# lastz/lastz

Measured on AMD Instinct MI355X. Metric: Gbp-of-target aligned/sec (whole job, --nogapped HSP path, both strands), higher is better.
Workload: dtype s32

## Files before the change

### lastz_amd/csrc/lz_lut.hpp

```cpp
#pragma once
#include "lz_common.hpp"

#define LZ_PAD2         128
#define LZ_LUT_ENTRIES  4096
#define LZ_LUT_TOTAL    (2 * LZ_LUT_ENTRIES)
#define LZ_LUT_WIN_G    15
#define LZ_LUT_WIN_B    60
#define LZ_LUT_MAXWIN   3
#define LZ_GRAY(c)      ((c) ^ ((c) >> 1))

struct alignas(8) LzLutEntry { u32 ab; u32 sc; };

struct LzLutParams {
    const u8* t2; const u8* q2;
    const u8* tsp; const u8* qsp;
    const u8* t2x; const u8* tspx;
    const u8* tcode; const u8* qcode;
    s32 xdrop;
};

struct LzLutScan { u32 s; s32 run, best; u32 room, used, alive, nwin; };

#if defined(__HIP_DEVICE_COMPILE__)
LZ_HD u32 lz_alignbit(u32 hi, u32 lo, u32 sh) { return __builtin_amdgcn_alignbit(hi, lo, sh); }
LZ_HD s32 lz_sdot4(u32 a, s32 acc) { return __builtin_amdgcn_sdot4((int)a, 0x01010101, acc, false); }
LZ_HD s32 lz_sdot4m(u32 a, u32 ones, s32 acc) { return __builtin_amdgcn_sdot4((int)a, (int)ones, acc, false); }
LZ_HD u32 lz_byte_pair(u32 hi_src, u32 lo_src, int k)
{ return __builtin_amdgcn_perm(hi_src, lo_src, 0x0C0C0000u | ((u32)(4 + k) << 8) | (u32)k); }
#define LZ_UNROLL_ALL _Pragma("unroll")
#else
LZ_HD u32 lz_alignbit(u32 hi, u32 lo, u32 sh) { sh &= 31u; return sh ? (lo >> sh) | (hi << (32u - sh)) : lo; }
LZ_HD s32 lz_sdot4(u32 a, s32 acc) { for (int k = 0; k < 4; k++) acc += (s32)(int8_t)(a >> (8 * k)); return acc; }
LZ_HD s32 lz_sdot4m(u32 a, u32 ones, s32 acc) { for (int k = 0; k < 4; k++) acc += (s32)(int8_t)(a >> (8 * k)) * (s32)((ones >> (8 * k)) & 0xFFu); return acc; }
LZ_HD u32 lz_byte_pair(u32 hi_src, u32 lo_src, int k) { return (((hi_src >> (8 * k)) & 0xFFu) << 8) | ((lo_src >> (8 * k)) & 0xFFu); }
#define LZ_UNROLL_ALL
#endif
LZ_HD u32 lz_ctz64(u64 x) { return (u32)__builtin_ctzll(x); }
LZ_HD u32 lz_clz64(u64 x) { return (u32)__builtin_clzll(x); }

template <bool SPECIAL> struct LzLutRaw { LzVec16 tv, qv, tm, qm; };
template <> struct LzLutRaw<false> { LzVec16 tv, qv; };
#define LZ_LUT_GBYTE(RIGHT_, g_) ((RIGHT_) ? (g_) : 14 - (g_))
template <bool RIGHT, bool SPECIAL>
LZ_HD void lz_lut_fetch(const LzLutParams& P, u32 s_, s32 diag, LzLutRaw<SPECIAL>& raw)
{
    const u32 st = RIGHT ? s_ + (u32)LZ_PAD2 : s_ - 1u + (u32)LZ_PAD2;
    const u32 sq = st - (u32)diag;
    const u32 back = RIGHT ? 0u : 15u;
    raw.tv = lz_load16(P.t2 + ((st >> 2) - back)); raw.qv = lz_load16(P.q2 + ((sq >> 2) - back));
    if constexpr (SPECIAL) {
        const u32 mback = RIGHT ? 0u : 14u;
        raw.tm = lz_load16(P.tsp + ((st >> 3) - mback)); raw.qm = lz_load16(P.qsp + ((sq >> 3) - mback));
    }
}
template <bool RIGHT>
LZ_HD u64 lz_lut_mask64(const LzVec16& v, s64 s)
{
    if (RIGHT) {
        const u32 k = (u32)((u64)(s + LZ_PAD2) & 7u);
        return ((u64)lz_alignbit(v.w[2], v.w[1], k) << 32) | lz_alignbit(v.w[1], v.w[0], k);
    }
    const u32 k = 17u + (u32)((u64)(s - 1 + LZ_PAD2) & 7u);
    return ((u64)lz_alignbit(v.w[3], v.w[2], k) << 32) | lz_alignbit(v.w[2], v.w[1], k);
}

template <bool RIGHT, bool SPECIAL, bool LIMCHK>
LZ_HD void lz_lut_window(const LzLutParams& P, const LzLutEntry* lut, s32 diag, LzLutScan& st, const LzLutRaw<SPECIAL>& raw, const s32* ctab = nullptr)
{
    const s32 X = P.xdrop;
    const LzLutEntry* const tab = lut + (RIGHT ? 0 : LZ_LUT_ENTRIES);
    const u32 spad = RIGHT ? st.s + (u32)LZ_PAD2 : st.s - 1u + (u32)LZ_PAD2, qpad = spad - (u32)diag;
    u32 tw[4], qw[4];
    {
        const u32 a = RIGHT ? 2u * (spad & 3u) : 2u * (spad & 3u) + 2u;
        const u32 b = RIGHT ? 2u * (qpad & 3u) : 2u * (qpad & 3u) + 2u;
        tw[0] = lz_alignbit(raw.tv.w[1], raw.tv.w[0], a); tw[1] = lz_alignbit(raw.tv.w[2], raw.tv.w[1], a); tw[2] = lz_alignbit(raw.tv.w[3], raw.tv.w[2], a); tw[3] = raw.tv.w[3] >> a;
        qw[0] = lz_alignbit(raw.qv.w[1], raw.qv.w[0], b); qw[1] = lz_alignbit(raw.qv.w[2], raw.qv.w[1], b); qw[2] = lz_alignbit(raw.qv.w[3], raw.qv.w[2], b); qw[3] = raw.qv.w[3] >> b;
    }
    u32 lim = st.room < (u32)LZ_LUT_WIN_B ? st.room : (u32)LZ_LUT_WIN_B;
    bool soft = false;
    if constexpr (SPECIAL) {
        const s64 s = (s64)st.s, sq = s - (s64)diag;
        const u64 sm = lz_lut_mask64<RIGHT>(raw.tm, s) | lz_lut_mask64<RIGHT>(raw.qm, sq);
        const u32 nsp = sm ? (RIGHT ? lz_ctz64(sm) : lz_clz64(sm)) : 64u;
        if (nsp < lim) { soft = true; lim = nsp; }
    }
    u32 xw[4], wc[4];
    LZ_UNROLL_ALL
    for (int k = 0; k < 4; k++) {
        xw[k] = tw[k] ^ qw[k];
        const u32 u = (tw[k] & 0x11111111u) | ((tw[k] >> 1) & 0x22222222u);
        wc[k] = (u | (u >> 2)) & 0x0F0F0F0Fu;
    }
    const u32 glim = lim >> 2;
    s32 run = st.run, m = run - st.best + X;
    u32 np = 0, fsc = 0;
#if !defined(LZ_LUT_NO_EARLY_EXIT) && defined(__HIP_DEVICE_COMPILE__)
    {
#define LZ_LUT_ENTRY_OF(g_) tab[lz_byte_pair(wc[LZ_LUT_GBYTE(RIGHT, g_) >> 2], xw[LZ_LUT_GBYTE(RIGHT, g_) >> 2], LZ_LUT_GBYTE(RIGHT, g_) & 3)]
        LzLutEntry ea = LZ_LUT_ENTRY_OF(0), eb = ea;
        LZ_UNROLL_ALL
        for (int g = 0; g < LZ_LUT_WIN_G; g += 2) {
            if (g + 1 < LZ_LUT_WIN_G) eb = LZ_LUT_ENTRY_OF(g + 1);
            if (m < (s32)(ea.ab & 0xFFFFu)) goto groups_done;
            if (LIMCHK && (u32)g >= glim) goto groups_done;
            { const s32 bq = (s32)ea.ab >> 16; m = lz_sdot4(ea.sc, m < bq ? m : bq); run = lz_sdot4(ea.sc, run); np = (u32)g + 1u; }
            if (g + 1 < LZ_LUT_WIN_G) {
                if (g + 2 < LZ_LUT_WIN_G) ea = LZ_LUT_ENTRY_OF(g + 2);
                if (m < (s32)(eb.ab & 0xFFFFu)) goto groups_done;
                if (LIMCHK && (u32)(g + 1) >= glim) goto groups_done;
                { const s32 bq = (s32)eb.ab >> 16; m = lz_sdot4(eb.sc, m < bq ? m : bq); run = lz_sdot4(eb.sc, run); np = (u32)g + 2u; }
            }
        }
        groups_done:
        fsc = (np & 1u) ? eb.sc : ea.sc;
#undef LZ_LUT_ENTRY_OF
    }
#else
    {
        bool dead = false;
        LZ_UNROLL_ALL
        for (int g = 0; g < LZ_LUT_WIN_G; g++) {
            const int by = LZ_LUT_GBYTE(RIGHT, g);
            const LzLutEntry e = tab[lz_byte_pair(wc[by >> 2], xw[by >> 2], by & 3)];
            if (!dead) fsc = e.sc;
            dead = dead | (m < (s32)(e.ab & 0xFFFFu));
            if (LIMCHK) dead = dead | ((u32)g >= glim);
            const s32 bq = (s32)e.ab >> 16;
            const s32 t = lz_sdot4(e.sc, m < bq ? m : bq);
            const s32 r2 = lz_sdot4(e.sc, run);
            m = dead ? m : t; run = dead ? run : r2; np += dead ? 0u : 1u;
        }
    }
#endif
    u32 r = 0;
    if (np < (u32)LZ_LUT_WIN_G) { r = lim - 4u * np; if (r > 4u) r = 4u; }
    s32 best = run - m + X;
    const u32 sc = fsc;
    bool stop = false; u32 j = 0;
    if (LIMCHK) {
        LZ_UNROLL_ALL
        for (u32 b = 0; b < 4; b++) {
            const bool on = !stop && b < r;
            const s32 nr = run + (s32)(int8_t)(sc >> (8u * b));
            run = on ? nr : run;
// ... 48 lines not shown
    diag = (s32)(u32)(key >> 32);
    const u32 pos1 = pos2 + (u32)diag;
    const s32 stopl = diag > 0 ? diag : 0;
    const s32 stopr = ((s32)tlen <= (s32)qlen + diag) ? (s32)tlen : (s32)qlen + diag;
    L.s = R.s = pos1; L.run = L.best = R.run = R.best = 0; L.used = R.used = 0; L.nwin = R.nwin = 0;
    L.room = (u32)((s32)pos1 - stopl); R.room = (u32)(stopr - (s32)pos1);
    L.alive = ((s32)pos1 > stopl) ? 1u : 0u; R.alive = ((s32)pos1 < stopr) ? 1u : 0u;
}

LZ_HD u32 lz_lut_summary(const LzLutScan& L, const LzLutScan& R, s32 min_score)
{
    u32 summ = (L.used & 0xFFu) | ((R.used & 0xFFu) << 8);
    if (L.alive || R.alive || L.best + R.best >= min_score) summ |= LZ_SUMM_SLOW;
    return summ;
}

template <bool SPECIAL>
LZ_HD u32 lz_lut_probe_hit(const LzLutParams& P, const LzLutEntry* lut, u32 tlen, u32 qlen, s32 min_score, u64 key, const s32* ctab = nullptr)
{
    s32 diag; LzLutScan L, R;
    lz_lut_init(key, tlen, qlen, diag, L, R);
    while (L.alive == 1 && L.nwin < (u32)LZ_LUT_MAXWIN) lz_lut_step<false, SPECIAL>(P, lut, diag, L, ctab);
    while (R.alive == 1 && R.nwin < (u32)LZ_LUT_MAXWIN) lz_lut_step<true, SPECIAL>(P, lut, diag, R, ctab);
    return lz_lut_summary(L, R, min_score);
}

LZ_HD u64 lz_hit_record(u64 key, u32 summ)
{
    const u32 pos2 = (u32)key, diag = (u32)(key >> 32);
    const bool slow = (summ & LZ_SUMM_SLOW) != 0;
    const u64 payload = slow ? (u64)(diag >> 16) : (u64)(summ & 0xFFFFu);
    return (u64)pos2 | ((u64)(diag & 0xFFu) << 31) | (payload << 39) | (slow ? (1ull << 63) : 0ull);
}
#define LZ_REC_TAG(r)     ((u32)((r) >> 55) & 0xFFu)
#define LZ_REC_UNTAG(r)   ((r) & ~(0xFFull << 55))
LZ_HD u64 lz_hit_record_tagged(u64 key, u32 summ) { return lz_hit_record(key, summ) | ((u64)((u32)(key >> 40) & 0xFFu) << 55); }

#define LZ_WCTX_BYTES 32
struct alignas(16) LzWctx { u32 w[LZ_WCTX_BYTES / 4]; };
LZ_HD u32 lz_wctx_first_byte(u32 pos1) { return ((pos1 - 1u + (u32)LZ_PAD2) >> 2) - 15u; }
LZ_HD u32 lz_wctx_right_offset(u32 pos1) { return ((pos1 + (u32)LZ_PAD2) >> 2) - lz_wctx_first_byte(pos1); }
LZ_HD LzWctx lz_wctx_make(const u8* two, u32 pos1) { LzWctx e; __builtin_memcpy(&e, two + lz_wctx_first_byte(pos1), LZ_WCTX_BYTES); return e; }
LZ_HD void lz_wctx_windows(const LzWctx& e, u32 pos1, LzVec16& tl, LzVec16& tr)
{
    const bool at16 = lz_wctx_right_offset(pos1) == 16u;
    LZ_UNROLL_ALL
    for (int k = 0; k < 4; k++) {
        tl.w[k] = e.w[k];
        const u32 at15 = lz_alignbit(e.w[4 + k], e.w[3 + k], 24u);
        tr.w[k] = at16 ? e.w[4 + k] : at15;
    }
}

#define LZ_REC_POS2(r)    ((u32)((r) & 0x7FFFFFFFu))
#define LZ_REC_LOW8(r)    ((u32)((r) >> 31) & 0xFFu)
#define LZ_REC_PAYLOAD(r) ((u32)((r) >> 39) & 0xFFFFu)
#define LZ_REC_SLOW(r)    ((u32)((r) >> 63))
LZ_HD u64 lz_rec_with_index(u64 r, u32 idx)
{ return (r & ~((0xFFull << 31) | (0x1Full << 55))) | ((u64)(idx & 0xFFu) << 31) | ((u64)((idx >> 8) & 0x1Fu) << 55); }
#define LZ_REC_INDEX(r)   (((u32)((r) >> 31) & 0xFFu) | (((u32)((r) >> 55) & 0x1Fu) << 8))

template <class Emit>
LZ_HD void lz_settle_record(const LzExtendParams& P, const s32* score_tab, u64 rec, u32 h ,
                            u32& dend, u64& n_ext, u64& n_bp, Emit&& emit)
{
    const u32 p2 = LZ_REC_POS2(rec);
    if (dend > p2 - P.seed_len) return;
    n_ext++;
    const u32 pay = LZ_REC_PAYLOAD(rec);
    if (!LZ_REC_SLOW(rec)) {
        const u32 room = p2 - dend, dlo = pay & 0xFFu, dext = pay >> 8;
        const u32 extent = p2 + dext;
        n_bp += (dlo < room ? dlo : room) + dext;
        if (extent > dend) dend = extent;
        return;
    }
    const s32 diag = (s32)((pay << 16) | h);
    dend = lz_reextend(P, score_tab, p2, diag, dend, n_bp, emit);
}
```

### lastz_amd/csrc/lzgpu_api.hip

```cpp
#include <hip/hip_runtime.h>
#include <stdarg.h>
#include <stdio.h>
#include <stdlib.h>
#include <string.h>
#include <math.h>
#include <algorithm>
#include <mutex>
#include <thread>
#include <atomic>
#include "lz_ctx.hpp"
#include "lz_host.hpp"
#include "lz_lut.hpp"


static LzCtx g_ctx;
static void lz_release_statics();
void lz_phase_clocks_print();
LzCtx& lz_ctx() { return g_ctx; }

static thread_local std::string t_last_error, t_last_error_out;
static std::mutex g_err_m;
int lz_fail(int code, const char* fmt, ...)
{
    char buf[512];
// ... 399 lines not shown
{
    LzCtx& c = g_ctx;
    if (!c.target.have_raw || !c.wstart.p) return lz_fail(LZGPU_ERR_STATE, "no table buffers");
    dev_ptr[0] = c.target.raw_base(); bytes[0] = c.geom.tlen;
    dev_ptr[1] = c.wstart.p;          bytes[1] = ((uint64_t)(1u << c.seed.weight) + 1) * 4;
    dev_ptr[2] = c.wpos.p;            bytes[2] = (uint64_t)c.num_words * 4;
    return 0;
}

extern "C" int lzgpu_table_commit(void)
{
    LzCtx& c = g_ctx;
    if (!c.target.have_raw || !c.wstart.p) return lz_fail(LZGPU_ERR_STATE, "no table buffers");
    { int rc = lz_bind_thread(); if (rc) return rc; }
    if (c.target.host.size() != c.geom.tlen) {
        c.target.host.resize(c.geom.tlen);
        if (c.geom.tlen) LZ_HIP(hipMemcpy(c.target.host.data(), c.target.raw_base(), c.geom.tlen, hipMemcpyDeviceToHost));
        c.target.code_key = 0; c.target.dp_key = 0;
    }
    c.table_gen++;
    c.have_table = true;
    return 0;
}

extern "C" int lzgpu_device_copy(void* dst, const void* src, uint64_t bytes)
{
    int rc = require_init(); if (rc) return rc;
    if (!bytes) return 0;
    LZ_HIP(hipMemcpyAsync(dst, src, bytes, hipMemcpyDeviceToDevice, g_ctx.stream));
    LZ_HIP(hipStreamSynchronize(g_ctx.stream));
    return 0;
}


#include <chrono>
struct HostProf {
    bool on; double t[16]; const char* names[16] = { nullptr }; int n = 0;
    std::chrono::steady_clock::time_point last;
    HostProf() { on = getenv("LZGPU_HOSTPROF") != nullptr; for (auto& x : t) x = 0; }
    void start() { if (on) last = std::chrono::steady_clock::now(); }
    void lap(int k, const char* name) {
        if (!on) return;
        auto now = std::chrono::steady_clock::now();
        t[k] += std::chrono::duration<double, std::milli>(now - last).count(); names[k] = name; if (k >= n) n = k + 1; last = now;
    }
    ~HostProf() { if (on) for (int k = 0; k < n; k++) if (names[k]) fprintf(stderr, "[lzgpu hostprof] %-28s %10.2f ms total\n", names[k], t[k]); }
};
static HostProf g_hp;


static int lz_wctx_prepare(LzCtx& c, bool& fused)
{
    if (c.wctx.p && c.wctx_gen == c.table_gen && c.wctx_code_key == c.target.code_key && c.target.code_key) return 0;
    const size_t need = (size_t)c.num_words * LZ_WCTX_BYTES;
    if (c.num_words == 0) { fused = false; return 0; }
    if (need > c.wctx.cap || !c.wctx.p) {
        size_t fr = 0, tot = 0;
        if (hipMemGetInfo(&fr, &tot) != hipSuccess || need > (fr + c.wctx.cap) / 2 || c.wctx.ensure(need) != 0) {
            (void)hipGetLastError(); c.last_error.clear();
            c.wctx_gen = 0; c.wctx_code_key = 0;
            fused = false;
            return 0;
        }
    }
    c.wctx_gen = 0; c.wctx_code_key = 0;
    int rc = lzk_wctx_build(c);
    if (rc) return rc;
    c.wctx_gen = c.table_gen; c.wctx_code_key = c.target.code_key;
    return 0;
}

static int seed_search(const lz_search_args* a, lz_hsp** out, uint64_t* n_out)
{
    int rc = require_init(); if (rc) return rc;
    LzCtx& c = g_ctx;
    if (!a || !out || !n_out || !a->sub) return lz_fail(LZGPU_ERR_ARG, "null argument");
    *out = nullptr; *n_out = 0;
    if (!c.have_table) return lz_fail(LZGPU_ERR_STATE, "lzgpu_table_prepare has not been called");

    g_hp.start();
    SeqSlot* qs;
    if (a->query) {
        if (a->qlen >= 0x7FFFFFFFu) return LZGPU_NH_SIZE;
        qs = lz_query_slot(c, -1, true);
        if ((rc = slot_upload(c, *qs, a->query, a->qlen, false))) return rc;
    } else {
        qs = a->query_slot < 0 ? nullptr : lz_query_slot(c, a->query_slot, false);
        if (!qs) return lz_fail(LZGPU_ERR_ARG, "query slot %d is empty", a->query_slot);
    }
    const u8* qhost = a->query ? a->query : qs->host.data();
    const u32 qlen = qs->len;
    u32 lo = a->start, hi = a->end ? a->end : qlen;
    if (hi <= lo) return lz_fail(LZGPU_ERR_ARG, "in seed_hit_search(), interval is void (%u-%u)", lo, hi);
    if (hi > qlen) return lz_fail(LZGPU_ERR_ARG, "in seed_hit_search(), interval end is bad (%u>%u)", hi, qlen);

    g_hp.lap(7, "query slot");
    static std::vector<s32> last_sub; static u8 rowc[256], colc[256]; static s32 tab[LZ_NCLASS * LZ_NCLASS];
    u8 cls[256];
    if (last_sub.size() != 65536 || memcmp(last_sub.data(), a->sub, 65536 * sizeof(s32)) != 0 || !c.score_tab.p) {
        last_sub.clear();
        if ((rc = lzh_score_classes(a->sub, rowc, colc, tab))) return rc;
        if ((rc = c.score_tab.ensure(sizeof(tab)))) return rc;
        LZ_HIP(hipMemcpyAsync(c.score_tab.p, tab, sizeof(tab), hipMemcpyHostToDevice, c.stream));
        LZ_HIP(hipStreamSynchronize(c.stream));
        last_sub.assign(a->sub, a->sub + 65536);
    }
    g_hp.lap(8, "score classes + table upload");
// ... 363 lines not shown
```

### lastz_amd/csrc/seed_kernels.hip

```cpp
#include <hip/hip_runtime.h>
#include <cstring>
#include <cstdio>
#include <rocprim/device/device_radix_sort.hpp>
#include <rocprim/device/device_scan.hpp>
#include <rocprim/iterator/transform_iterator.hpp>
#include "lz_ctx.hpp"
#include "lz_lut.hpp"
#include "lz_tile_runs.hpp"
#include "lz_coop.hpp"

#define LZ_TPB 256

#if defined(LZ_NO_NT)
#define LZ_NT_LD(p_) (*(p_))
#define LZ_NT_ST(v_, p_) (*(p_) = (v_))
#else
#define LZ_NT_LD(p_) __builtin_nontemporal_load(p_)
#define LZ_NT_ST(v_, p_) __builtin_nontemporal_store((v_), (p_))
#endif
__global__ void __launch_bounds__(LZ_TPB)
k_encode(const u8* __restrict__ raw, u8* __restrict__ code, u32 len, const u8* __restrict__ cls)
{
    __shared__ u8 tab[256];
    tab[threadIdx.x] = cls[threadIdx.x];
// ... 673 lines not shown
    bin_base[threadIdx.x] = bb;
    for (u32 b = 0; b < nblocks; b++) part[(size_t)b * LZ_NBIN + threadIdx.x] += bb;
}

int lzk_hist_scan(LzCtx& c, u64 n, u32* hist, u32* part, u32* bin_base, hipStream_t st)
{
    const u32 ntiles = (u32)((n + LZ_PP_TILE - 1) / LZ_PP_TILE), nblocks = (ntiles + 255u) / 256u;
    c.timer.begin("k_hist_scan", st);
    if (nblocks) hipLaunchKernelGGL(k_hist_scan1, dim3(nblocks), dim3(LZ_NBIN), 0, st, hist, ntiles, part);
    hipLaunchKernelGGL(k_hist_scan2, dim3(1), dim3(LZ_NBIN), 0, st, part, nblocks, bin_base);
    c.timer.end(st);
    LZ_HIP(hipGetLastError());
    return 0;
}

__device__ __forceinline__ void lz_match8(u32 key, bool valid, u32 lane, u32& rank, u32& count, bool& last)
{
    u64 peers = __ballot(valid);
#pragma unroll
    for (int b = 0; b < 8; b++) {
        const bool bit = ((key >> b) & 1u) != 0;
        const u64 m = __ballot(bit && valid);
        peers &= bit ? m : ~m;
    }
    const u64 below = (1ull << lane) - 1ull;
    rank = (u32)__popcll(peers & below);
    count = (u32)__popcll(peers);
    last = (peers >> lane) == 1ull;
}
__device__ __forceinline__ u32 lz_exscan256(u32 v, u32* wtot )
{
    const u32 tid = threadIdx.x, lane = tid & 63u, w = tid >> 6;
    u32 inc = v;
#pragma unroll
    for (int d = 1; d < 64; d <<= 1) { const u32 t = __shfl_up(inc, d); if ((int)lane >= d) inc += t; }
    if (tid < 256 && lane == 63) wtot[w] = inc;
    __syncthreads();
    u32 pre = 0;
    if (tid < 256) for (u32 k = 0; k < w; k++) pre += wtot[k];
    return pre + inc - v;
}

struct LzScanTask { u32 idx; s32 diag; LzLutScan L, R; };
static_assert(sizeof(LzScanTask) == 64, "LzScanTask: one 64-byte line per task");
#define LZ_SC_TPB 512
template <int MODE> struct LzScanShared {
    union {
        LzLutEntry lut[LZ_LUT_TOTAL];
        struct { s32 tab[LZ_NCLASS * LZ_NCLASS]; s32 tab8[64]; } bc;
    };
    s32 ctab[MODE == 1 ? LZ_NCLASS * LZ_NCLASS : 1];
};

template <bool SP>
__device__ __forceinline__ void lz_scan_round(const LzExtendParams& P, const LzLutParams& Q, const LzLutEntry* lut, const s32* ctab, u64 key, bool valid,
                                              const LzLutRaw<SP>& rawl, const LzLutRaw<SP>& rawr, u32 idx, u32 lane,
                                              u32& summ_out, LzScanTask* __restrict__ my_tasks, u32& my_n, u32 region_cap)
{
    constexpr bool HLIM = SP;
    s32 diag; LzLutScan L, R;
    lz_lut_init(key, P.tlen, P.qlen, diag, L, R);
    if (!valid) { L.alive = 0; R.alive = 0; }
    const bool ql = L.alive && !HLIM && L.room < (u32)LZ_LUT_WIN_B, qr = R.alive && !HLIM && R.room < (u32)LZ_LUT_WIN_B;
    lz_lut_window_pair<SP, HLIM>(Q, lut, diag, L, R, rawl, rawr, L.alive && !ql, R.alive && !qr, ctab);
    const bool more = valid && (L.alive == 1 || R.alive == 1);
    const u64 mm = __ballot(more);
    bool queued = false;
    if (mm) {
        const u32 slot = my_n + (u32)__popcll(mm & ((1ull << lane) - 1ull));
        if (more && slot < region_cap) {
            LzScanTask t; t.idx = idx; t.diag = diag; t.L = L; t.R = R;
            my_tasks[slot] = t; queued = true;
        }
        my_n += (u32)__popcll(mm);
    }
    summ_out = queued ? 0u : lz_lut_summary(L, R, P.min_score);
}
template <bool SP>
__device__ __forceinline__ void lz_scan_fetch(const LzLutParams& Q, u64 key, LzLutRaw<SP>& rawl, LzLutRaw<SP>& rawr)
{
    const u32 pos2 = (u32)key, pos1 = pos2 + (u32)(key >> 32);
    const s32 diag = (s32)(u32)(key >> 32);
    const u32 stl = pos1 - 1u + (u32)LZ_PAD2, str = pos1 + (u32)LZ_PAD2;
    const u32 bl = (stl >> 2) - 15u, br = str >> 2;
    const u32 ol = bl + (bl & ~31u);
    rawl.tv = lz_load16(Q.t2x + ol); rawr.tv = lz_load16(Q.t2x + (ol + (br - bl)));
    const u32 sql = stl - (u32)diag, sqr = str - (u32)diag;
    rawl.qv = lz_load16(Q.q2 + ((sql >> 2) - 15u)); rawr.qv = lz_load16(Q.q2 + (sqr >> 2));
    if constexpr (SP) {
        const u32 ml = (stl >> 3) - 14u, mr = str >> 3;
        const u32 oml = ml + (ml & ~31u);
        rawl.tm = lz_load16(Q.tspx + oml); rawr.tm = lz_load16(Q.tspx + (oml + (mr - ml)));
        rawl.qm = lz_load16(Q.qsp + ((sql >> 3) - 14u)); rawr.qm = lz_load16(Q.qsp + (sqr >> 3));
    }
}

template <int MODE, int TPB, int WPE>
__global__ void __launch_bounds__(TPB, WPE)
k_scan_hits(LzExtendParams P, LzLutParams Q, const u64* __restrict__ keys, u64 n,
            const s32* __restrict__ score_tab_g, const LzLutEntry* __restrict__ lut_g,
            u32* __restrict__ summ, u8* __restrict__ bins, LzScanTask* __restrict__ tasks, u32* __restrict__ n_tasks, u32 region_cap)
{
    __shared__ LzScanShared<MODE> sh;
    const u32 tid = threadIdx.x, lane = tid & 63u, w = tid >> 6;
    if (MODE == 1) { for (u32 k = tid; k < LZ_NCLASS * LZ_NCLASS; k += TPB) sh.ctab[k] = score_tab_g[k]; }
    if (MODE < 2) { for (u32 k = tid; k < LZ_LUT_TOTAL; k += TPB) sh.lut[k] = lut_g[k]; }
    else {
        for (u32 k = tid; k < LZ_NCLASS * LZ_NCLASS; k += TPB) sh.bc.tab[k] = score_tab_g[k];
        if (tid < 64) sh.bc.tab8[tid] = score_tab_g[(tid >> 3) * LZ_NCLASS + (tid & 7)];
    }
    __syncthreads();
    const LzLutEntry* lut = sh.lut;
    const s32* const ctab = sh.ctab;
    constexpr bool SP = MODE == 1;
    constexpr u32 SPAN = 64u * LZ_SC_ROUNDS;
    static_assert(LZ_SC_ROUNDS == 4, "the round pipeline below is written out for four rounds per span");
// ... 190 lines not shown
    if ((rc = c.summ[set].ensure((size_t)max_n * 4))) return rc;
    if (mode < 2 && (rc = c.scan_tasks[set].ensure((size_t)n_regions * region_cap * sizeof(LzScanTask)))) return rc;
    return c.scan_ntasks[set].ensure((size_t)n_regions * 4);
}

int lzk_scan_hits(LzCtx& c, int set, int mode, const LzExtendParams& P, const LzLutParams& Q, const u64* keys, u64 n,
                  const s32* score_tab, const LzLutEntry* lut, u8* bins, hipStream_t st)
{
    if (n == 0) return 0;
    int cus = 256; (void)hipDeviceGetAttribute(&cus, hipDeviceAttributeMultiprocessorCount, c.device);
    int rc;
    u32 grid, n_regions, task_cap;
    lz_scan_geometry(c, mode, n, grid, n_regions, task_cap);
    if ((rc = c.summ[set].ensure((size_t)n * 4))) return rc;
    if (mode < 2 && (rc = c.scan_tasks[set].ensure((size_t)n_regions * task_cap * sizeof(LzScanTask)))) return rc;
    if ((rc = c.scan_ntasks[set].ensure((size_t)n_regions * 4))) return rc;
    u32* summ = c.summ[set].as<u32>(); LzScanTask* tasks = c.scan_tasks[set].as<LzScanTask>(); u32* ntk = c.scan_ntasks[set].as<u32>();
    c.timer.begin("k_scan_hits", st);
    const int tpb = lz_scan_tpb(mode);
#define LZ_SCAN_LAUNCH(M_, T_, W_) hipLaunchKernelGGL((k_scan_hits<M_, T_, W_>), dim3(grid), dim3(T_), 0, st, P, Q, keys, n, score_tab, lut, summ, bins, tasks, ntk, task_cap)
    if (mode == 0) {
        if (tpb == 640)       LZ_SCAN_LAUNCH(0, 640, 5);
        else if (tpb == 768)  LZ_SCAN_LAUNCH(0, 768, 6);
        else if (tpb == 1024) LZ_SCAN_LAUNCH(0, 1024, 8);
        else                  LZ_SCAN_LAUNCH(0, 512, 4);
    }
    else if (mode == 1) LZ_SCAN_LAUNCH(1, LZ_SC_TPB, 4);
    else                LZ_SCAN_LAUNCH(2, LZ_SC_TPB, 4);
#undef LZ_SCAN_LAUNCH
    c.timer.end(st);
    LZ_HIP(hipGetLastError());
    if (mode < 2) {
        c.timer.begin("k_scan_tasks", st);
        if (mode == 0) hipLaunchKernelGGL(k_scan_tasks<0>, dim3(std::min<u32>(n_regions, 4u * (u32)cus)), dim3(LZ_ST_TPB), 0, st, P, Q, lut, score_tab, tasks, ntk, n_regions, task_cap, summ);
        else           hipLaunchKernelGGL(k_scan_tasks<1>, dim3(std::min<u32>(n_regions, 4u * (u32)cus)), dim3(LZ_ST_TPB), 0, st, P, Q, lut, score_tab, tasks, ntk, n_regions, task_cap, summ);
        c.timer.end(st);
        LZ_HIP(hipGetLastError());
    }
    return 0;
}

int lzk_partition(LzCtx& c, int set, u64* keys, u64 n, u32* hist, u32* run_addr, hipStream_t st)
{
    if (n == 0) return 0;
    const u32 ntiles = (u32)((n + LZ_PP_TILE - 1) / LZ_PP_TILE);
    c.timer.begin("k_partition", st);
    hipLaunchKernelGGL(k_partition, dim3(ntiles), dim3(LZ_PP_TPB), 0, st, keys, c.summ[set].as<u32>(), n, hist, run_addr, keys);
    c.timer.end(st);
    LZ_HIP(hipGetLastError());
    return 0;
}

__global__ void __launch_bounds__(LZ_TPB)
k_build_wctx(const u32* __restrict__ wpos, u64 num_words, const u8* __restrict__ two, LzVec16* __restrict__ wctx)
{
    const u64 j = (u64)blockIdx.x * LZ_TPB + threadIdx.x;
    if (j >= 2 * num_words) return;
    const u32 pos1 = wpos[j >> 1];
    wctx[j] = lz_load16(two + lz_wctx_first_byte(pos1) + 16u * (u32)(j & 1u));
}

template <int CAP> struct LzFuse2Wave {
    alignas(16) u32 own32[CAP / 2];
    u32 lsrc[64 * LZ_FILL_GROUP];
    uint2 ent[64];
};
struct LzFuseTrip { u32 p1, pos2, dst; bool ok; LzWctx cx; LzVec16 ql, qr; };

template <bool SELF, int TPB, int CAP>
__global__ void __launch_bounds__(TPB)
k_scan_hits2(u32 lo, u32 i0, u32 i1, LzSeedDev sd,
             const u32* __restrict__ wstart, const u32* __restrict__ wpos, const LzWctx* __restrict__ wctx,
             const u32* __restrict__ sk, const u32* __restrict__ sv, u32 n, const u64* __restrict__ off, u64 base,
             LzExtendParams P, LzLutParams Q, const LzLutEntry* __restrict__ lut_g,
             u64* __restrict__ recs, LzScanTask* __restrict__ tasks, u32* __restrict__ n_tasks, u32 region_cap, LzSelfDev self)
{
    static_assert(CAP % 512 == 0, "whole 16-byte groups of own[] per lane");
    constexpr int WORDS = CAP / 2 / 64;
    __shared__ LzLutEntry lut[LZ_LUT_TOTAL];
    __shared__ LzFuse2Wave<CAP> shw[TPB / 64];
    for (u32 k = threadIdx.x; k < LZ_LUT_TOTAL; k += TPB) lut[k] = lut_g[k];
    __syncthreads();
    LzFuse2Wave<CAP>& sh = shw[threadIdx.x >> 6];
    unsigned short* const own = reinterpret_cast<unsigned short*>(sh.own32);
    const u32 lane = threadIdx.x & 63u;
    const u32 region = blockIdx.x * (TPB / 64) + (threadIdx.x >> 6), nwaves = gridDim.x * (TPB / 64);
    LzScanTask* const my_tasks = tasks + (size_t)region * region_cap;
    u32 my_n = 0;
    const u32 ngroups = (n + 63u) / 64u;
    for (u32 grp = region; grp < ngroups; grp += nwaves) {
        const u32 j = grp * 64u + lane;
        u32 w_l = 0, i_l = 0; bool in = false;
        if (j < n) { w_l = sk[j] & ((2u << sd.weight) - 1u); i_l = sv[j]; in = !(w_l >> sd.weight) && i_l >= i0 && i_l < i1; }
        if (!__ballot(in)) continue;
        const u32 dbase = in ? (u32)(off[i_l] - base) : 0u;
        const u32 pos2 = lo + i_l + 1u;
        u32 slo = 0, shi = 0;
        if (SELF) lz_self_bounds(self, pos2, slo, shi);
        u32 carry = 0;
        for (int r = 0; r < sd.nprobes; r += LZ_FILL_GROUP) {
            u32 la[LZ_FILL_GROUP], len[LZ_FILL_GROUP]; u32 total = 0;
#pragma unroll
            for (int p = 0; p < LZ_FILL_GROUP; p++) {
                const bool on = in && r + p < sd.nprobes;
                const u32 w = on ? (w_l ^ sd.probe_xor[(r + p) & (LZ_MAX_PROBES - 1)]) : 0u;
                la[p] = wstart[w]; len[p] = wstart[w + 1];
            }
#pragma unroll
            for (int p = 0; p < LZ_FILL_GROUP; p++) {
                const bool on = in && r + p < sd.nprobes;
                len[p] = on ? len[p] - la[p] : 0u;
                if (!SELF) total += len[p];
            }
            if (SELF) {
                lz_clip_runs<LZ_FILL_GROUP>(wpos, la, len, slo, shi);
#pragma unroll
                for (int p = 0; p < LZ_FILL_GROUP; p++) total += len[p];
            }
            u32 inc = total;
            LZ_WAVE_SCAN_U32(inc, total, lz_uadd)
            const u32 E = inc - total;
            const u32 T = (u32)__builtin_amdgcn_readlane((int)inc, 63);
            {
                u32 S = E;
#pragma unroll
                for (int p = 0; p < LZ_FILL_GROUP; p++) { sh.lsrc[lane * LZ_FILL_GROUP + p] = la[p] - S; S += len[p]; }
            }
            sh.ent[lane] = make_uint2(dbase + carry - E, pos2);
            for (u32 cs = 0; cs < T; cs += CAP) {
                const u32 tc = (T - cs < (u32)CAP) ? T - cs : (u32)CAP;
                uint4* const mine = reinterpret_cast<uint4*>(sh.own32 + lane * WORDS);
#pragma unroll
                for (int k = 0; k < WORDS / 4; k++) mine[k] = make_uint4(0u, 0u, 0u, 0u);
                __atomic_signal_fence(__ATOMIC_SEQ_CST);
                {
                    u32 S = E;
#pragma unroll
                    for (int p = 0; p < LZ_FILL_GROUP; p++) {
                        const u32 l = len[p];
                        if (l && S < cs + tc && S + l > cs) own[(S > cs ? S : cs) - cs] = (unsigned short)(1u + lane * LZ_FILL_GROUP + (u32)p);
                        S += l;
                    }
                }
                __atomic_signal_fence(__ATOMIC_SEQ_CST);
                u32 wv[WORDS];
#pragma unroll
                for (int k = 0; k < WORDS / 4; k++) { const uint4 v = mine[k]; wv[4 * k] = v.x; wv[4 * k + 1] = v.y; wv[4 * k + 2] = v.z; wv[4 * k + 3] = v.w; }
                u32 segmax = 0;
#pragma unroll
                for (int k = 0; k < WORDS; k++) { const u32 m2 = lz_umax(wv[k] & 0xFFFFu, wv[k] >> 16); segmax = lz_umax(segmax, m2); }
                u32 sinc = segmax;
                LZ_WAVE_SCAN_U32(sinc, segmax, lz_umax)
                u32 run = lz_dpp_u32<0x138, 0xf, 0xf>(0u, sinc);
#pragma unroll
                for (int k = 0; k < WORDS; k++) {
                    const u32 a0 = lz_umax(wv[k] & 0xFFFFu, run), a1 = lz_umax(wv[k] >> 16, a0);
                    wv[k] = a0 | (a1 << 16); run = a1;
                }
#pragma unroll
                for (int k = 0; k < WORDS / 4; k++) mine[k] = make_uint4(wv[4 * k], wv[4 * k + 1], wv[4 * k + 2], wv[4 * k + 3]);
                __atomic_signal_fence(__ATOMIC_SEQ_CST);
                auto load_trip = [&](u32 tb, LzFuseTrip& t) {
                    const u32 t0 = tb + lane;
                    t.ok = t0 < tc;
                    const u32 tt = t.ok ? t0 : tc - 1u;
                    const u32 list = (u32)own[tt] - 1u;
                    const u32 ls = sh.lsrc[list];
                    const uint2 en = sh.ent[list / LZ_FILL_GROUP];
                    const u32 tabs = cs + tt, e = ls + tabs;
                    t.p1 = wpos[e]; t.cx = wctx[e];
                    t.pos2 = en.y; t.dst = en.x + tabs;
                    const u32 sql = en.y - 1u + (u32)LZ_PAD2;
                    t.ql = lz_load16(Q.q2 + ((sql >> 2) - 15u)); t.qr = lz_load16(Q.q2 + ((sql + 1u) >> 2));
                };
                auto scan_trip = [&](const LzFuseTrip& t) {
                    const u64 key = lz_hit_key(t.p1, t.pos2);
                    LzLutRaw<false> rl, rr;
                    lz_wctx_windows(t.cx, t.p1, rl.tv, rr.tv);
                    rl.qv = t.ql; rr.qv = t.qr;
                    u32 summ;
                    lz_scan_round<false>(P, Q, lut, nullptr, key, t.ok, rl, rr, t.dst, lane, summ, my_tasks, my_n, region_cap);
                    if (t.ok) LZ_NT_ST(lz_hit_record_tagged(key, summ), recs + t.dst);
                };
                LzFuseTrip ta, tb2;
                load_trip(0u, ta);
#pragma unroll 1
                for (u32 tb = 0;;) {
                    if (tb + 64u < tc) load_trip(tb + 64u, tb2);
                    scan_trip(ta);
                    tb += 64u; if (tb >= tc) break;
                    if (tb + 64u < tc) load_trip(tb + 64u, ta);
                    scan_trip(tb2);
                    tb += 64u; if (tb >= tc) break;
                }
                __atomic_signal_fence(__ATOMIC_SEQ_CST);
            }
            carry += total;
        }
    }
    if (lane == 0) n_tasks[region] = my_n < region_cap ? my_n : region_cap;
}

__global__ void __launch_bounds__(LZ_ST_TPB)
k_scan_tasks2(LzExtendParams P, LzLutParams Q, const LzLutEntry* __restrict__ lut_g, const LzScanTask* __restrict__ tasks,
              const u32* __restrict__ n_tasks, u32 n_regions, u32 region_cap, u64* __restrict__ recs)
{
    __shared__ LzLutEntry lut[LZ_LUT_TOTAL];
    for (u32 k = threadIdx.x; k < LZ_LUT_TOTAL; k += LZ_ST_TPB) lut[k] = lut_g[k];
    __syncthreads();
    for (u32 region = blockIdx.x; region < n_regions; region += gridDim.x) {
        const u32 nt = n_tasks[region];
        for (u32 k = threadIdx.x; k < nt; k += (u32)LZ_ST_TPB) {
            const LzScanTask t = tasks[(size_t)region * region_cap + k];
            LzLutScan L = t.L, R = t.R;
            const u32 pos1 = L.alive == 1 ? L.s + (u32)LZ_LUT_WIN_B * L.nwin : R.s - (u32)LZ_LUT_WIN_B * R.nwin;
            while (L.alive == 1 && L.nwin < (u32)LZ_LUT_MAXWIN) lz_lut_step<false, false>(Q, lut, t.diag, L, nullptr);
            while (R.alive == 1 && R.nwin < (u32)LZ_LUT_MAXWIN) lz_lut_step<true, false>(Q, lut, t.diag, R, nullptr);
            recs[t.idx] = lz_hit_record_tagged(lz_hit_key(pos1, pos1 - (u32)t.diag), lz_lut_summary(L, R, P.min_score));
        }
    }
}

__global__ void __launch_bounds__(LZ_PP_TPB)
k_partition2(u64* recs, u64 n, u32* __restrict__ hist, u32* __restrict__ run_addr)
{
    __shared__ LzPartShared sh;
    const u32 tid = threadIdx.x, lane = tid & 63u, w = tid >> 6;
    const u32 tile = blockIdx.x;
    const u64 base = (u64)tile * LZ_PP_TILE;
    const u32 tile_n = (n - base < (u64)LZ_PP_TILE) ? (u32)(n - base) : (u32)LZ_PP_TILE;
    for (u32 k = tid; k < LZ_PP_WAVES * LZ_NBIN; k += LZ_PP_TPB) { (&sh.wcnt[0][0])[k] = 0; (&sh.bm[0][0])[k] = 0ull; }
    const u32 l0 = w * (64u * LZ_PP_ROUNDS) + lane;
    u64 rr[LZ_PP_ROUNDS];
#pragma unroll
    for (u32 r = 0; r < LZ_PP_ROUNDS; r++) rr[r] = (l0 + 64u * r < tile_n) ? recs[base + l0 + 64u * r] : 0ull;
    __syncthreads();
#define LZ_PART_BIN(r_) LZ_REC_TAG(rr[r_])
    LZ_PART_RANKS(LZ_PART_BIN)
#undef LZ_PART_BIN
#pragma unroll
    for (u32 r = 0; r < LZ_PP_ROUNDS; r++) {
        const u32 bin = LZ_REC_TAG(rr[r]);
        if (l0 + 64u * r < tile_n) sh.stage[sh.tstart[bin] + sh.wcnt[w][bin] + slot[r]] = rr[r];
    }
    __syncthreads();
    lz_part_store(sh.stage, tile_n, recs + base);
}

int lzk_wctx_build(LzCtx& c)
{
    const u64 nw = c.num_words;
    if (nw == 0) return 0;
    c.timer.begin("k_build_wctx", c.stream);
    hipLaunchKernelGGL(k_build_wctx, dim3((unsigned)((2 * nw + LZ_TPB - 1) / LZ_TPB)), dim3(LZ_TPB), 0, c.stream,
                       c.wpos.as<u32>(), nw, c.target.two.as<u8>(), c.wctx.as<LzVec16>());
    c.timer.end(c.stream);
    LZ_HIP(hipGetLastError());
    return 0;
}

static u32 lz_fused_tpb(LzCtx& c)
{
    static const int env = getenv("LZGPU_FUSE_TPB") ? atoi(getenv("LZGPU_FUSE_TPB")) : 0;
    if (c.self.mode != LZ_SELF_OFF) return 512u;
    return (env == 512 || env == 768 || env == 1024) ? (u32)env : 1024u;
}
static void lz_fused_geometry(LzCtx& c, u64 n_hits, u32& grid, u32& n_regions, u32& region_cap)
{
    int cus = 256; (void)hipDeviceGetAttribute(&cus, hipDeviceAttributeMultiprocessorCount, c.device);
    grid = (u32)cus; n_regions = grid * (lz_fused_tpb(c) / 64u);
    region_cap = (u32)std::min<u64>(n_hits / 32 / n_regions + 64, 1u << 20);
    static const char* force = getenv("LZGPU_TASK_REGION_CAP");
    if (force && atoi(force) > 0) region_cap = (u32)atoi(force);
}
int lzk_fused_reserve(LzCtx& c, int set, u64 max_n)
{
    u32 grid, n_regions, region_cap; int rc;
    lz_fused_geometry(c, max_n, grid, n_regions, region_cap);
    if ((rc = c.scan_tasks[set].ensure((size_t)n_regions * region_cap * sizeof(LzScanTask)))) return rc;
    return c.scan_ntasks[set].ensure((size_t)n_regions * 4);
}
int lzk_scan_fused(LzCtx& c, int set, u32 lo, u32 i0, u32 i1, const u32* sk, const u32* sv, u32 n, const u64* off, u64 base, u64 n_hits,
                   const LzExtendParams& P, const LzLutParams& Q, const LzLutEntry* lut, u64* tagged, hipStream_t st)
{
    if (n == 0 || i1 <= i0 || n_hits == 0) return 0;
    if (!c.blk_start_host.empty()) {
        const u32 b0 = i0 >> c.blk_shift, b1 = (i1 - 1) >> c.blk_shift;
        const u64 j0 = c.blk_start_host[b0], j1 = c.blk_start_host[std::min<u32>(b1 + 1, c.blk_count)];
        sk += j0; sv += j0; n = (u32)(j1 - j0);
        if (n == 0) return 0;
    }
    int rc;
    u32 grid, n_regions, region_cap;
    lz_fused_geometry(c, n_hits, grid, n_regions, region_cap);
    if ((rc = c.scan_tasks[set].ensure((size_t)n_regions * region_cap * sizeof(LzScanTask)))) return rc;
    if ((rc = c.scan_ntasks[set].ensure((size_t)n_regions * 4))) return rc;
    LzScanTask* tasks = c.scan_tasks[set].as<LzScanTask>(); u32* ntk = c.scan_ntasks[set].as<u32>();
    c.timer.begin("k_scan_hits", st);
    const u32 tpb = lz_fused_tpb(c);
#define LZ_FUSED_LAUNCH(S_, T_, C_, self_) hipLaunchKernelGGL((k_scan_hits2<S_, T_, C_>), dim3(grid), dim3(T_), 0, st, lo, i0, i1, c.seed, c.wstart.as<u32>(), c.wpos.as<u32>(), \
                           c.wctx.as<LzWctx>(), sk, sv, n, off, base, P, Q, lut, tagged, tasks, ntk, region_cap, self_)
    if (c.self.mode != LZ_SELF_OFF) LZ_FUSED_LAUNCH(true, 512, 2560, c.self);
    else if (tpb == 512)            LZ_FUSED_LAUNCH(false, 512, 2560, LzSelfDev{});
    else if (tpb == 768)            LZ_FUSED_LAUNCH(false, 768, 1024, LzSelfDev{});
    else                            LZ_FUSED_LAUNCH(false, 1024, 512, LzSelfDev{});
#undef LZ_FUSED_LAUNCH
    c.timer.end(st);
    LZ_HIP(hipGetLastError());
    c.timer.begin("k_scan_tasks", st);
    hipLaunchKernelGGL(k_scan_tasks2, dim3(std::min<u32>(n_regions, 4u * grid)), dim3(LZ_ST_TPB), 0, st, P, Q, lut, tasks, ntk, n_regions, region_cap, tagged);
    c.timer.end(st);
    LZ_HIP(hipGetLastError());
    return 0;
}
int lzk_partition_tagged(LzCtx& c, u64* tagged, u64 n, u32* hist, u32* run_addr, hipStream_t st)
{
    if (n == 0) return 0;
    const u32 ntiles = (u32)((n + LZ_PP_TILE - 1) / LZ_PP_TILE);
    c.timer.begin("k_partition", st);
    hipLaunchKernelGGL(k_partition2, dim3(ntiles), dim3(LZ_PP_TPB), 0, st, tagged, n, hist, run_addr);
    c.timer.end(st);
    LZ_HIP(hipGetLastError());
    return 0;
}

__device__ __forceinline__ LzCoopMap lz_coop_shfl_up32(const LzCoopMap& v, int d)
{ LzCoopMap r; r.A = __shfl_up(v.A, d, 32); r.B = __shfl_up(v.B, d, 32); r.C = __shfl_up(v.C, d, 32); return r; }
__device__ LzCoopSide lz_coop_extend_wave(const LzExtendParams& P, const s32* tab, u32 pos1, s32 diag, s32 stopl, s32 stopr, u32 lane)
{
    const s32 X = P.xdrop;
    const bool right = lane >= 32u;
    const u32 hl = lane & 31u;
    const s32 stop = right ? stopr : stopl;
    LzCoopSide out; out.stop_pos = pos1; out.best_pos = pos1; out.best = 0;
    s32 run0 = 0, best0 = 0; u32 s = pos1;
    bool alive = (right ? ((s32)s < stop) : ((s32)s > stop)) && X >= 0;
    while (__ballot(alive)) {
        const u32 room = alive ? (right ? (u32)(stop - (s32)s) : (u32)((s32)s - stop)) : 0u;
        const u32 off = LZ_COOP_BLK * hl;
        const u32 nb = room > off ? (room - off < (u32)LZ_COOP_BLK ? room - off : (u32)LZ_COOP_BLK) : 0u;
        s32 sc[LZ_COOP_BLK];
        {
            LzVec16 tv = { { 0, 0, 0, 0 } }, qv = { { 0, 0, 0, 0 } };
            if (nb) {
                const s64 t0 = right ? (s64)s + off : (s64)s - off - LZ_COOP_BLK;
                tv = lz_load16(P.tcode + t0); qv = lz_load16(P.qcode + (t0 - diag));
            }
#pragma unroll
            for (int j = 0; j < LZ_COOP_BLK; j++) {
                const u32 tb = right ? LZ_VBYTE(tv, j) : LZ_VBYTE(tv, LZ_COOP_BLK - 1 - j);
                const u32 qb = right ? LZ_VBYTE(qv, j) : LZ_VBYTE(qv, LZ_COOP_BLK - 1 - j);
                sc[j] = tab[(LZ_CODE_CLASS(tb) << 5) | LZ_CODE_CLASS(qb)];
            }
        }
// ... 363 lines not shown
```

Before: 0.4044.

## Precompute aligned target words and class planes per target word in wctx table

The per-word target context table now stores the target windows already shifted into alignment for the left and right extensions, plus packed nibble class planes, in 48 bytes instead of 32 raw bytes. The fused scan kernel skips the per-hit window extraction, target alignbit shifts and plane computation, and only aligns the query side. In exchange the precomputed table is larger, so each trip loads more bytes and holds more register state, and the build kernel does more work per word.

```diff
diff --git a/lastz_amd/csrc/lz_lut.hpp b/lastz_amd/csrc/lz_lut.hpp
--- a/lastz_amd/csrc/lz_lut.hpp
+++ b/lastz_amd/csrc/lz_lut.hpp
@@ -64,18 +64,27 @@
     return ((u64)lz_alignbit(v.w[3], v.w[2], k) << 32) | lz_alignbit(v.w[2], v.w[1], k);
 }
 
-template <bool RIGHT, bool SPECIAL, bool LIMCHK>
-LZ_HD void lz_lut_window(const LzLutParams& P, const LzLutEntry* lut, s32 diag, LzLutScan& st, const LzLutRaw<SPECIAL>& raw, const s32* ctab = nullptr)
+template <bool RIGHT> LZ_HD u32 lz_lut_shift(u32 spad) { return RIGHT ? 2u * (spad & 3u) : 2u * (spad & 3u) + 2u; }
+LZ_HD void lz_lut_align(const LzVec16& v, u32 a, u32 w[4])
+{ w[0] = lz_alignbit(v.w[1], v.w[0], a); w[1] = lz_alignbit(v.w[2], v.w[1], a); w[2] = lz_alignbit(v.w[3], v.w[2], a); w[3] = v.w[3] >> a; }
+LZ_HD u32 lz_lut_plane(u32 tw) { const u32 u = (tw & 0x11111111u) | ((tw >> 1) & 0x22222222u); return (u | (u >> 2)) & 0x0F0F0F0Fu; }
+
+struct LzWprep;
+template <bool RIGHT> LZ_HD void lz_wprep_words(const LzWprep& e, u32 (&tw)[4], u32 (&wc)[4]);
+template <bool RIGHT, bool SPECIAL, bool LIMCHK, bool PREP = false>
+LZ_HD void lz_lut_window(const LzLutParams& P, const LzLutEntry* lut, s32 diag, LzLutScan& st, const LzLutRaw<SPECIAL>& raw, const s32* ctab = nullptr,
+                         const LzWprep* prep = nullptr)
 {
     const s32 X = P.xdrop;
     const LzLutEntry* const tab = lut + (RIGHT ? 0 : LZ_LUT_ENTRIES);
     const u32 spad = RIGHT ? st.s + (u32)LZ_PAD2 : st.s - 1u + (u32)LZ_PAD2, qpad = spad - (u32)diag;
-    u32 tw[4], qw[4];
-    {
-        const u32 a = RIGHT ? 2u * (spad & 3u) : 2u * (spad & 3u) + 2u;
-        const u32 b = RIGHT ? 2u * (qpad & 3u) : 2u * (qpad & 3u) + 2u;
-        tw[0] = lz_alignbit(raw.tv.w[1], raw.tv.w[0], a); tw[1] = lz_alignbit(raw.tv.w[2], raw.tv.w[1], a); tw[2] = lz_alignbit(raw.tv.w[3], raw.tv.w[2], a); tw[3] = raw.tv.w[3] >> a;
-        qw[0] = lz_alignbit(raw.qv.w[1], raw.qv.w[0], b); qw[1] = lz_alignbit(raw.qv.w[2], raw.qv.w[1], b); qw[2] = lz_alignbit(raw.qv.w[3], raw.qv.w[2], b); qw[3] = raw.qv.w[3] >> b;
+    u32 tw[4], qw[4], wc[4];
+    if constexpr (PREP) {
+        lz_wprep_words<RIGHT>(*prep, tw, wc);
+        lz_lut_align(raw.qv, lz_lut_shift<RIGHT>(qpad), qw);
+    } else {
+        const u32 a = lz_lut_shift<RIGHT>(spad), b = lz_lut_shift<RIGHT>(qpad);
+        lz_lut_align(raw.tv, a, tw); lz_lut_align(raw.qv, b, qw);
     }
     u32 lim = st.room < (u32)LZ_LUT_WIN_B ? st.room : (u32)LZ_LUT_WIN_B;
     bool soft = false;
@@ -85,12 +94,11 @@
         const u32 nsp = sm ? (RIGHT ? lz_ctz64(sm) : lz_clz64(sm)) : 64u;
         if (nsp < lim) { soft = true; lim = nsp; }
     }
-    u32 xw[4], wc[4];
+    u32 xw[4];
     LZ_UNROLL_ALL
     for (int k = 0; k < 4; k++) {
         xw[k] = tw[k] ^ qw[k];
-        const u32 u = (tw[k] & 0x11111111u) | ((tw[k] >> 1) & 0x22222222u);
-        wc[k] = (u | (u >> 2)) & 0x0F0F0F0Fu;
+        if constexpr (!PREP) wc[k] = lz_lut_plane(tw[k]);
     }
     const u32 glim = lim >> 2;
     s32 run = st.run, m = run - st.best + X;
@@ -245,6 +253,35 @@
     }
 }
 
+#define LZ_WPREP_BYTES 48
+struct alignas(16) LzWprep { u32 tl[4], tr[4], pk[4]; };
+static_assert(sizeof(LzWprep) == LZ_WPREP_BYTES, "LzWprep: three 16-byte loads");
+LZ_HD LzWprep lz_wprep_make(const u8* two, u32 pos1)
+{
+    const LzWctx raw = lz_wctx_make(two, pos1);
+    LzVec16 vl, vr;
+    lz_wctx_windows(raw, pos1, vl, vr);
+    LzWprep e;
+    lz_lut_align(vl, lz_lut_shift<false>(pos1 - 1u + (u32)LZ_PAD2), e.tl);
+    lz_lut_align(vr, lz_lut_shift<true>(pos1 + (u32)LZ_PAD2), e.tr);
+    LZ_UNROLL_ALL
+    for (int k = 0; k < 4; k++) e.pk[k] = lz_lut_plane(e.tl[k]) | (lz_lut_plane(e.tr[k]) << 4);
+    return e;
+}
+template <bool RIGHT>
+LZ_HD void lz_wprep_words(const LzWprep& e, u32 (&tw)[4], u32 (&wc)[4])
+{
+    LZ_UNROLL_ALL
+    for (int k = 0; k < 4; k++) { tw[k] = RIGHT ? e.tr[k] : e.tl[k]; wc[k] = (RIGHT ? e.pk[k] >> 4 : e.pk[k]) & 0x0F0F0F0Fu; }
+}
+template <bool RIGHT>
+LZ_HD void lz_lut_window_prep(const LzLutParams& P, const LzLutEntry* lut, s32 diag, LzLutScan& st, const LzWprep& e, const LzVec16& qv)
+{
+    LzLutRaw<false> raw;
+    raw.tv = LzVec16{{0u, 0u, 0u, 0u}}; raw.qv = qv;
+    lz_lut_window<RIGHT, false, false, true>(P, lut, diag, st, raw, nullptr, &e);
+}
+
 #define LZ_REC_POS2(r)    ((u32)((r) & 0x7FFFFFFFu))
 #define LZ_REC_LOW8(r)    ((u32)((r) >> 31) & 0xFFu)
 #define LZ_REC_PAYLOAD(r) ((u32)((r) >> 39) & 0xFFFFu)
diff --git a/lastz_amd/csrc/lzgpu_api.hip b/lastz_amd/csrc/lzgpu_api.hip
--- a/lastz_amd/csrc/lzgpu_api.hip
+++ b/lastz_amd/csrc/lzgpu_api.hip
@@ -475,7 +475,7 @@
 static int lz_wctx_prepare(LzCtx& c, bool& fused)
 {
     if (c.wctx.p && c.wctx_gen == c.table_gen && c.wctx_code_key == c.target.code_key && c.target.code_key) return 0;
-    const size_t need = (size_t)c.num_words * LZ_WCTX_BYTES;
+    const size_t need = (size_t)c.num_words * LZ_WPREP_BYTES;
     if (c.num_words == 0) { fused = false; return 0; }
     if (need > c.wctx.cap || !c.wctx.p) {
         size_t fr = 0, tot = 0;
diff --git a/lastz_amd/csrc/seed_kernels.hip b/lastz_amd/csrc/seed_kernels.hip
--- a/lastz_amd/csrc/seed_kernels.hip
+++ b/lastz_amd/csrc/seed_kernels.hip
@@ -749,16 +749,21 @@
     s32 ctab[MODE == 1 ? LZ_NCLASS * LZ_NCLASS : 1];
 };
 
-template <bool SP>
+template <bool SP, bool PREP = false>
 __device__ __forceinline__ void lz_scan_round(const LzExtendParams& P, const LzLutParams& Q, const LzLutEntry* lut, const s32* ctab, u64 key, bool valid,
                                               const LzLutRaw<SP>& rawl, const LzLutRaw<SP>& rawr, u32 idx, u32 lane,
-                                              u32& summ_out, LzScanTask* __restrict__ my_tasks, u32& my_n, u32 region_cap)
+                                              u32& summ_out, LzScanTask* __restrict__ my_tasks, u32& my_n, u32 region_cap, const LzWprep* prep = nullptr)
 {
     constexpr bool HLIM = SP;
     s32 diag; LzLutScan L, R;
     lz_lut_init(key, P.tlen, P.qlen, diag, L, R);
     if (!valid) { L.alive = 0; R.alive = 0; }
     const bool ql = L.alive && !HLIM && L.room < (u32)LZ_LUT_WIN_B, qr = R.alive && !HLIM && R.room < (u32)LZ_LUT_WIN_B;
+    if constexpr (PREP) {
+        static_assert(!SP, "prepared windows: mode 0");
+        if (L.alive && !ql) lz_lut_window<false, false, false, true>(Q, lut, diag, L, rawl, nullptr, prep);
+        if (R.alive && !qr) lz_lut_window<true, false, false, true>(Q, lut, diag, R, rawr, nullptr, prep);
+    } else
     lz_lut_window_pair<SP, HLIM>(Q, lut, diag, L, R, rawl, rawr, L.alive && !ql, R.alive && !qr, ctab);
     const bool more = valid && (L.alive == 1 || R.alive == 1);
     const u64 mm = __ballot(more);
@@ -1055,12 +1060,11 @@
 }
 
 __global__ void __launch_bounds__(LZ_TPB)
-k_build_wctx(const u32* __restrict__ wpos, u64 num_words, const u8* __restrict__ two, LzVec16* __restrict__ wctx)
-{
-    const u64 j = (u64)blockIdx.x * LZ_TPB + threadIdx.x;
-    if (j >= 2 * num_words) return;
-    const u32 pos1 = wpos[j >> 1];
-    wctx[j] = lz_load16(two + lz_wctx_first_byte(pos1) + 16u * (u32)(j & 1u));
+k_build_wctx(const u32* __restrict__ wpos, u64 num_words, const u8* __restrict__ two, LzWprep* __restrict__ wctx)
+{
+    const u64 e = (u64)blockIdx.x * LZ_TPB + threadIdx.x;
+    if (e >= num_words) return;
+    wctx[e] = lz_wprep_make(two, wpos[e]);
 }
 
 template <int CAP> struct LzFuse2Wave {
@@ -1068,12 +1072,12 @@
     u32 lsrc[64 * LZ_FILL_GROUP];
     uint2 ent[64];
 };
-struct LzFuseTrip { u32 p1, pos2, dst; bool ok; LzWctx cx; LzVec16 ql, qr; };
+struct LzFuseTrip { u32 p1, pos2, dst; bool ok; LzWprep cx; LzVec16 ql, qr; };
 
 template <bool SELF, int TPB, int CAP>
 __global__ void __launch_bounds__(TPB)
 k_scan_hits2(u32 lo, u32 i0, u32 i1, LzSeedDev sd,
-             const u32* __restrict__ wstart, const u32* __restrict__ wpos, const LzWctx* __restrict__ wctx,
+             const u32* __restrict__ wstart, const u32* __restrict__ wpos, const LzWprep* __restrict__ wctx,
              const u32* __restrict__ sk, const u32* __restrict__ sv, u32 n, const u64* __restrict__ off, u64 base,
              LzExtendParams P, LzLutParams Q, const LzLutEntry* __restrict__ lut_g,
              u64* __restrict__ recs, LzScanTask* __restrict__ tasks, u32* __restrict__ n_tasks, u32 region_cap, LzSelfDev self)
@@ -1179,10 +1183,9 @@
                 auto scan_trip = [&](const LzFuseTrip& t) {
                     const u64 key = lz_hit_key(t.p1, t.pos2);
                     LzLutRaw<false> rl, rr;
-                    lz_wctx_windows(t.cx, t.p1, rl.tv, rr.tv);
-                    rl.qv = t.ql; rr.qv = t.qr;
+                    rl.tv = rl.qv = t.ql; rr.tv = rr.qv = t.qr;
                     u32 summ;
-                    lz_scan_round<false>(P, Q, lut, nullptr, key, t.ok, rl, rr, t.dst, lane, summ, my_tasks, my_n, region_cap);
+                    lz_scan_round<false, true>(P, Q, lut, nullptr, key, t.ok, rl, rr, t.dst, lane, summ, my_tasks, my_n, region_cap, &t.cx);
                     if (t.ok) LZ_NT_ST(lz_hit_record_tagged(key, summ), recs + t.dst);
                 };
                 LzFuseTrip ta, tb2;
@@ -1255,8 +1258,8 @@
     const u64 nw = c.num_words;
     if (nw == 0) return 0;
     c.timer.begin("k_build_wctx", c.stream);
-    hipLaunchKernelGGL(k_build_wctx, dim3((unsigned)((2 * nw + LZ_TPB - 1) / LZ_TPB)), dim3(LZ_TPB), 0, c.stream,
-                       c.wpos.as<u32>(), nw, c.target.two.as<u8>(), c.wctx.as<LzVec16>());
+    hipLaunchKernelGGL(k_build_wctx, dim3((unsigned)((nw + LZ_TPB - 1) / LZ_TPB)), dim3(LZ_TPB), 0, c.stream,
+                       c.wpos.as<u32>(), nw, c.target.two.as<u8>(), c.wctx.as<LzWprep>());
     c.timer.end(c.stream);
     LZ_HIP(hipGetLastError());
     return 0;
@@ -1302,7 +1305,7 @@
     c.timer.begin("k_scan_hits", st);
     const u32 tpb = lz_fused_tpb(c);
 #define LZ_FUSED_LAUNCH(S_, T_, C_, self_) hipLaunchKernelGGL((k_scan_hits2<S_, T_, C_>), dim3(grid), dim3(T_), 0, st, lo, i0, i1, c.seed, c.wstart.as<u32>(), c.wpos.as<u32>(), \
-                           c.wctx.as<LzWctx>(), sk, sv, n, off, base, P, Q, lut, tagged, tasks, ntk, region_cap, self_)
+                           c.wctx.as<LzWprep>(), sk, sv, n, off, base, P, Q, lut, tagged, tasks, ntk, region_cap, self_)
     if (c.self.mode != LZ_SELF_OFF) LZ_FUSED_LAUNCH(true, 512, 2560, c.self);
     else if (tpb == 512)            LZ_FUSED_LAUNCH(false, 512, 2560, LzSelfDev{});
     else if (tpb == 768)            LZ_FUSED_LAUNCH(false, 768, 1024, LzSelfDev{});
```

Result: no change. 0.4085 (median of 6 runs) (+1.0%).
